# SunBangjie/FYP-BidirectionalPathTracer

Hardware: AMD Instinct MI355X
Metric: Mrays/s + RMSE vs the scalar oracle, BDPT pass, Sponza-class scene 1920x1080 depth 8 (higher is better)
Workload: dtype f32

## Files before the change

### fyp-bidirectionalpathtracer_amd/csrc/api.cpp

```cpp
#include <hip/hip_runtime.h>

#include <cmath>
#include <cstdio>
#include <cstdlib>
#include <cstring>
#include <future>
#include <functional>
#include <atomic>
#include <chrono>
#include <string>
#include <thread>
#include <vector>

#include "../../include/bdpt.h"
#include <new>

#include "bvh.h"
#include "kernels.h"
#include "refit.h"
#include "scene_bvh.h"

using namespace bdpt;

namespace {
// ... 440 lines not shown
    up(&u.shade, shade.data(), shade.size());
    up(&u.indices, d->indices, (size_t)d->numTriangles * 3);
    if (d->bitangents) up(&u.bitangents, d->bitangents, (size_t)d->numVertices * 3);
    return u;
  });
  struct SideJoin {
    std::future<SideUploads>& f;
    ~SideJoin() {
      if (!f.valid()) return;
      try {
        SideUploads u = f.get();
        for (void* q : u.pool) (void)hipFree(q);
      } catch (...) {
      }
    }
  } sideJoin{side};
  SceneBvh sb;
  try {
    std::string treeError;
    struct Build {
      BvhDeviceBuild* b;
      ~Build() { bvhDeviceBuildEnd(b); }
    } build{bvhDeviceBuildBegin(c->device, std::getenv("BDPT_HOST_COLLAPSE") == nullptr)};
    buildSceneBvh(d, 0, -1.0f, -1.0f, std::getenv("BDPT_NO_ALPHA_CLASSIFY") == nullptr, sb, buildBinaryTreeOnDevice, build.b, &treeError, packOnDevice, makeReferencesOnDevice,
                  std::getenv("BDPT_HOST_COLLAPSE") == nullptr, std::getenv("BDPT_HOST_PRIORITIES") == nullptr);
    if (sb.bvh.deviceRecs) c->sceneAllocs.push_back(sb.bvh.deviceRecs);
    if (!treeError.empty()) {
      fail(c, "scene: " + treeError);
      return treeError.find("2^31") != std::string::npos ? BDPT_E_LIMIT : (treeError.find("out of device memory") != std::string::npos ? BDPT_E_NOMEM : BDPT_E_HIP);
    }
  } catch (const std::bad_alloc&) {
    fail(c, "scene: out of host memory while building the acceleration structure");
    return BDPT_E_NOMEM;
  }
  lap("buildSceneBvh");
  Bvh& bvh = sb.bvh;
  const std::vector<uint32_t>& alphaTris = sb.alphaTris;
  if (bvh.maxStack > (uint32_t)kBvhMaxStack) {
    fail(c, "bvh needs a deeper traversal stack than the device provides");
    return BDPT_E_LIMIT;
  }
  if (!bvh.deviceRecs && !bvh.recs.empty()) {
    const BvhRec* dRecs = nullptr;
    if (int rc0 = devUpload(c, c->sceneAllocs, &dRecs, bvh.recs.data(), bvh.recs.size())) return rc0;
    bvh.deviceRecs = const_cast<BvhRec*>(dRecs);
    bvh.deviceNumRecs = bvh.recs.size();
  }
  if (!bvh.deviceRecs) {
    fail(c, "scene: the acceleration structure has no records");
    return BDPT_E_HIP;
  }
  c->bvhInfo.numNodes = bvh.numNodes;
  c->bvhInfo.numTriangles = d->numTriangles;
  c->bvhInfo.maxDepth = bvh.maxDepth;
  c->bvhInfo.nodeBytes = sizeof(BvhRec);
  c->bvhInfo.triBytes = sizeof(BvhTri);
  c->bvhInfo.sahCost = bvh.sahCost;
  c->bvhInfo.maxStack = bvh.maxStack;
  c->bvhInfo.numReferences = bvh.numRefs;
  c->bvhInfo.numDropped = bvh.numDropped;
  c->bvhInfo.numAlphaMode = sb.numAlphaMode;
  c->bvhInfo.numAlwaysPass = sb.numAlwaysPass;

  int rc;
  {
    SideUploads u = side.get();
    c->sceneAllocs.insert(c->sceneAllocs.end(), u.pool.begin(), u.pool.end());
    if (u.err != hipSuccess) {
      fail(c, std::string("scene upload: ") + (u.what.empty() ? std::string(hipGetErrorString(u.err)) : u.what));
      return u.err == hipErrorOutOfMemory ? BDPT_E_NOMEM : BDPT_E_HIP;
    }
    c->S.shade = reinterpret_cast<const float4*>(u.shade);
    c->S.indices = u.indices;
    if (d->bitangents) {
      c->S.bitangents = u.bitangents;
      c->S.hasBitangents = 1;
    }
  }
  lap("shading records + uploads (joined)");
  c->S.recs = reinterpret_cast<const uint4*>(bvh.deviceRecs);
  c->S.numRecs = (uint32_t)bvh.deviceNumRecs;
  if ((rc = devUpload(c, c->sceneAllocs, &c->S.materials, d->materials, d->numMaterials))) return rc;
  std::vector<TexDev> texs(d->numTextures);
  for (uint32_t i = 0; i < d->numTextures; i++) {
    const bdpt_texture& t = d->textures[i];
    if (!t.rgba8 || !t.width || !t.height) {
      fail(c, "scene: empty texture");
      return BDPT_E_INVALID;
    }
    const size_t bytes = (size_t)t.width * t.height * 4;
    uint8_t* px = nullptr;
    if ((rc = devAlloc(c, c->sceneAllocs, &px, bytes + 4))) return rc;
    HIPCHK(c, hipMemset(px + bytes, 0, 4));
    {
      std::string e;
      if (!bvhUploadStaged(px, t.rgba8, bytes, e)) {
        fail(c, e);
        return BDPT_E_HIP;
      }
    }
    texs[i] = TexDev{px, t.width, t.height, t.srgb, texPow2Flags(t.width, t.height)};
  }
  if ((rc = devUpload(c, c->sceneAllocs, &c->S.textures, texs.data(), texs.size()))) return rc;
  {
    std::vector<TexDev> matTex((size_t)d->numMaterials * 4, TexDev{nullptr, 0, 0, 0, 0});
    for (uint32_t mi = 0; mi < d->numMaterials; mi++) {
      const bdpt_material& mm = d->materials[mi];
      const int ids[4] = {mm.texBaseColor, mm.texSpecular, mm.texEmissive, mm.texNormal};
      for (int k = 0; k < 4; k++)
        if (ids[k] >= 0) matTex[(size_t)mi * 4 + k] = texs[(size_t)ids[k]];
    }
    if ((rc = devUpload(c, c->sceneAllocs, &c->S.matTex, matTex.data(), matTex.size()))) return rc;
  }
  {
    float4* dAlpha = nullptr;
    if ((rc = devAlloc(c, c->sceneAllocs, &dAlpha, std::max<size_t>(alphaTris.size(), 1) * 4))) return rc;
    if (alphaTris.empty()) {
      HIPCHK(c, hipMemset(dAlpha, 0, 4 * sizeof(float4)));
    } else {
      std::vector<uint8_t> alphaMat(d->numMaterials, 0);
      for (const uint32_t t : alphaTris) alphaMat[d->triMaterial[t]] = 1;
      std::vector<unsigned long long> quadByTex(std::max<size_t>(d->numTextures, 1), 0ull);
      for (uint32_t mi = 0; mi < d->numMaterials; mi++) {
        const bdpt_material& mm = d->materials[mi];
        if (!alphaMat[mi] || !alphaSamplesTexture(BDPT_FLAG_DIFFUSE_TYPE(mm.flags), mm.texBaseColor) || quadByTex[(size_t)mm.texBaseColor])
          continue;
        const std::vector<uint32_t> plane = alphaQuadPlane(d->textures[mm.texBaseColor]);
        const uint32_t* dPlane = nullptr;
        if ((rc = devUpload(c, c->sceneAllocs, &dPlane, plane.data(), plane.size()))) return rc;
        quadByTex[(size_t)mm.texBaseColor] = (unsigned long long)reinterpret_cast<uintptr_t>(dPlane);
      }
      const uint32_t* dList = nullptr;
      const unsigned long long* dQuad = nullptr;
      std::vector<void*> scratch;
      if ((rc = devUpload(c, c->sceneAllocs, &dList, alphaTris.data(), alphaTris.size())) ||
          (rc = devUpload(c, scratch, &dQuad, quadByTex.data(), quadByTex.size()))) {
        freePool(scratch);
        return rc;
      }
      c->alphaTris = dList;
      c->numAlphaTris = (uint32_t)alphaTris.size();
      launchAlphaRecs(c->S, dList, (uint32_t)alphaTris.size(), dQuad, dAlpha, nullptr);
      const hipError_t e = hipDeviceSynchronize();
      freePool(scratch);
      HIPCHK(c, e);
    }
    c->S.alphaRecs = dAlpha;
  }
  lap("indices, textures, alpha");
  SceneConst sc;
  std::memset(&sc, 0, sizeof(sc));
  std::memcpy(sc.lights, d->lights, sizeof(bdpt_light) * d->numLights);
  for (int i = 0; i < 256; i++) {
    double cc = (double)i / 255.0;
    double l = (cc <= 0.04045) ? cc / 12.92 : std::pow((cc + 0.055) / 1.055, 2.4);
    sc.srgbLut[i] = (float)l;
  }
  if ((rc = devUpload(c, c->sceneAllocs, &c->S.sc, &sc, 1))) return rc;
  c->S.numLights = d->numLights;
  c->hints = std::getenv("BDPT_NO_HINTS") == nullptr;
  if (c->hints) {
    uint32_t res = 512;
    if (const char* e = std::getenv("BDPT_LIGHT_MAP_RES")) res = (uint32_t)std::max(0, std::min(2048, std::atoi(e)));
    if (res) {
      uint32_t* maps = nullptr;
      if ((rc = devAlloc(c, c->sceneAllocs, &maps, (size_t)6 * res * res * d->numLights))) return rc;
      launchLightMaps(c->S, maps, res, nullptr);
      HIPCHK(c, hipDeviceSynchronize());
      c->S.lightMap = maps;
      c->S.lightMapRes = res;
      c->lightMaps = maps;
    }
  }
  if (c->hintPix) HIPCHK(c, hipMemset(c->hintPix, 0xFF, (size_t)c->W * c->H * sizeof(uint32_t)));
  c->hintCamValid = false;
  lap("light maps");
  c->numVertices = d->numVertices;
  c->numTriangles = d->numTriangles;
  c->haveScene = true;
  return BDPT_OK;
}
int bdpt_set_scene(bdpt_ctx* c, const bdpt_scene_desc* d) {
  try {
    return setSceneImpl(c, d);
  } catch (const std::bad_alloc&) {
    fail(c, "scene: out of host memory while building the acceleration structure");
    return BDPT_E_NOMEM;
  } catch (const std::exception& e) {
    fail(c, std::string("scene: ") + e.what());
    return BDPT_E_INVALID;
  }
}


int bdpt_get_bvh_info(const bdpt_ctx* c, bdpt_bvh_info* out) {
  if (!c || !out) return BDPT_E_INVALID;
  if (!c->haveScene) return BDPT_E_STATE;
  *out = c->bvhInfo;
  return BDPT_OK;
}

int bdpt_set_camera(bdpt_ctx* c, const bdpt_camera* cam) {
  if (!c || !cam) return BDPT_E_INVALID;
  c->cam = *cam;
  c->haveCamera = true;
  return BDPT_OK;
}

int bdpt_set_environment(bdpt_ctx* c, const bdpt_environment* env) {
  if (!c) return BDPT_E_INVALID;
  if (env && env->envMap && (!env->width || !env->height)) {
    fail(c, "environment: a map needs a width and a height");
    return BDPT_E_INVALID;
  }
  c->env = env ? *env : bdpt_environment{};
  if (!c->env.envMap) c->env.width = c->env.height = 0;
  return BDPT_OK;
}

namespace {
int ensureRefit(bdpt_ctx* c, hipStream_t st) {
  if (c->refitReady) return BDPT_OK;
  if (streamIsCapturing(st)) {
    fail(c, "update: the first update needs bdpt_prepare(BDPT_PREPARE_REFIT) before stream capture");
    return BDPT_E_STATE;
  }
  HIPCHK(c, hipDeviceSynchronize());
  BvhRefitPlan plan;
  {
    std::vector<BvhRec> recs(c->S.numRecs);
    HIPCHK(c, hipMemcpy(recs.data(), c->S.recs, recs.size() * sizeof(BvhRec), hipMemcpyDeviceToHost));
    std::string err;
    if (!bvhRefitMakePlan(recs.data(), recs.size(), plan, err)) {
      fail(c, err);
      return BDPT_E_HIP;
    }
  }
  const size_t nn = std::max<size_t>(plan.nodes.size(), 1);
  RefitDev R{};
  const BvhRefitNode* dNodes = nullptr;
// ... 1440 lines not shown
```

### fyp-bidirectionalpathtracer_amd/csrc/device_scene.hpp

```cpp
#pragma once
#include "device_math.hpp"
#include "kernels.h"

namespace bdpt {
#define BD __device__ __forceinline__

struct f4 {
  float x, y, z, w;
};
BD f4 lerp4(f4 a, f4 b, float s) {
  return f4{a.x + (b.x - a.x) * s, a.y + (b.y - a.y) * s, a.z + (b.z - a.z) * s, a.w + (b.w - a.w) * s};
}
typedef __attribute__((address_space(1))) const uint32_t gU32;
typedef __attribute__((address_space(1), aligned(4))) const unsigned long long gU64a4;
BD void texelRow(const uint8_t* px, uint32_t w, int iy, int ix0, int ix1, uint32_t& a, uint32_t& b) {
  gU32* row = (gU32*)px + (size_t)iy * w;
  const unsigned long long q = *(gU64a4*)(row + ix0);
  a = (uint32_t)q;
  b = (uint32_t)(q >> 32);
  if (ix1 != ix0 + 1) b = row[ix1];
}
BD f4 texel(const SceneDev& S, const TexDev& t, uint32_t p) {
  f4 r;
  if (t.srgb) {
    r.x = S.sc->srgbLut[p & 0xffu];
    r.y = S.sc->srgbLut[(p >> 8) & 0xffu];
    r.z = S.sc->srgbLut[(p >> 16) & 0xffu];
  } else {
    r.x = (float)(p & 0xffu) / 255.0f;
    r.y = (float)((p >> 8) & 0xffu) / 255.0f;
    r.z = (float)((p >> 16) & 0xffu) / 255.0f;
  }
  r.w = (float)(p >> 24) / 255.0f;
  return r;
}
BD f4 sampleBilinearT(const SceneDev& S, const TexDev& t, float u, float v) {
  float x = u * (float)t.w - 0.5f;
  float y = v * (float)t.h - 0.5f;
  float x0 = floorf(x), y0 = floorf(y);
  float fx = x - x0, fy = y - y0;
  int ix0 = wrapT((int)x0, (int)t.w, (t.pow2 & kTexPow2W) != 0u), iy0 = wrapT((int)y0, (int)t.h, (t.pow2 & kTexPow2H) != 0u);
  int ix1 = wrapNext(ix0, (int)t.w), iy1 = wrapNext(iy0, (int)t.h);
  uint32_t p00, p10, p01, p11;
  texelRow(t.px, t.w, iy0, ix0, ix1, p00, p10);
  texelRow(t.px, t.w, iy1, ix0, ix1, p01, p11);
  f4 t00 = texel(S, t, p00), t10 = texel(S, t, p10);
  f4 t01 = texel(S, t, p01), t11 = texel(S, t, p11);
  return lerp4(lerp4(t00, t10, fx), lerp4(t01, t11, fx), fy);
}
BD f4 sampleBilinear(const SceneDev& S, int texId, float u, float v) { return sampleBilinearT(S, S.textures[texId], u, v); }
BD f4 sampleTexture(const SceneDev& S, int texId, float u, float v, f4 factor, uint32_t mode) {
  if (mode == BDPT_CHANNEL_UNUSED) return f4{0, 0, 0, 0};
  if (mode == BDPT_CHANNEL_CONST || texId < 0) return factor;
  return sampleBilinear(S, texId, u, v);
}
BD f4 sampleTextureT(const SceneDev& S, const TexDev& t, int texId, float u, float v, f4 factor, uint32_t mode) {
  if (mode == BDPT_CHANNEL_UNUSED) return f4{0, 0, 0, 0};
  if (mode == BDPT_CHANNEL_CONST || texId < 0) return factor;
  return sampleBilinearT(S, t, u, v);
}

struct MatDev {
  f4 baseColor, specular;
  f3 emissive;
  float alphaThreshold, IoR;
  uint32_t flags;
  int texBase, texSpec, texEmis, texNorm;
};
BD MatDev loadMaterial(const SceneDev& S, uint32_t id) {
  const float4* m = reinterpret_cast<const float4*>(S.materials + id);
  float4 a = m[0], b = m[1], c = m[2], d = m[3];
  MatDev r;
  r.baseColor = f4{a.x, a.y, a.z, a.w};
  r.specular = f4{b.x, b.y, b.z, b.w};
  r.emissive = mk(c.x, c.y, c.z);
  r.alphaThreshold = c.w;
  r.IoR = d.x;
  r.flags = __float_as_uint(d.y);
  uint32_t t0 = __float_as_uint(d.z), t1 = __float_as_uint(d.w);
  r.texBase = (int)(int16_t)(t0 & 0xffffu);
  r.texSpec = (int)(int16_t)(t0 >> 16);
  r.texEmis = (int)(int16_t)(t1 & 0xffffu);
  r.texNorm = (int)(int16_t)(t1 >> 16);
  return r;
}

BD uint32_t alphaQuad(const float4& a2, const float4& a3, float u, float v, float& fx, float& fy) {
  const int tw = (int)__float_as_uint(a2.y), th = (int)__float_as_uint(a2.z);
  const uint32_t pow2 = __float_as_uint(a2.w);
  gU32* px = (gU32*)(((unsigned long long)__float_as_uint(a3.y) << 32) | (unsigned long long)__float_as_uint(a3.x));
  const float x = u * (float)tw - 0.5f, y = v * (float)th - 0.5f;
  const float x0 = floorf(x), y0 = floorf(y);
  fx = x - x0;
  fy = y - y0;
  const int ix0 = wrapT((int)x0, tw, (pow2 & kTexPow2W) != 0u), iy0 = wrapT((int)y0, th, (pow2 & kTexPow2H) != 0u);
  return px[(size_t)iy0 * tw + (size_t)ix0];
}
BD bool alphaTestFails(const SceneDev& S, uint32_t rec, float bu, float bv) {
  const float4* r = S.alphaRecs + (size_t)rec * 4;
  const float4 a0 = r[0], a1 = r[1], a2 = r[2], a3 = r[3];
  const uint32_t mode = __float_as_uint(a2.x);
  float alpha = 0.0f;
  if (mode == 1u) {
    alpha = a1.w;
  } else if (mode == 2u) {
    float u = 0, v = 0;
    const float b0 = 1.0f - bu - bv;
    u += a0.x * b0;
    v += a0.y * b0;
    u += a0.z * bu;
    v += a0.w * bu;
    u += a1.x * bv;
    v += a1.y * bv;
    float fx, fy;
    const uint32_t q = alphaQuad(a2, a3, u, v, fx, fy);
    const float t00 = (float)(q & 0xffu) / 255.0f, t10 = (float)((q >> 8) & 0xffu) / 255.0f;
    const float t01 = (float)((q >> 16) & 0xffu) / 255.0f, t11 = (float)(q >> 24) / 255.0f;
    const float top = t00 + (t10 - t00) * fx, bot = t01 + (t11 - t01) * fx;
    alpha = top + (bot - top) * fy;
  }
  return alpha < a1.z;
}

struct AlphaIn {
  float4 a0, a1, a2, a3;
};
BD void alphaTexels(const AlphaIn& r, float bu, float bv, bool run, float& fx, float& fy, float& t00, float& t10, float& t01, float& t11) {
  fx = fy = t00 = t10 = t01 = t11 = 0.0f;
  if (!run || __float_as_uint(r.a2.x) != 2u) return;
  float u = 0, v = 0;
  const float b0 = 1.0f - bu - bv;
  u += r.a0.x * b0;
  v += r.a0.y * b0;
  u += r.a0.z * bu;
  v += r.a0.w * bu;
  u += r.a1.x * bv;
  v += r.a1.y * bv;
  const uint32_t q = alphaQuad(r.a2, r.a3, u, v, fx, fy);
  t00 = (float)(q & 0xffu);
  t10 = (float)((q >> 8) & 0xffu);
  t01 = (float)((q >> 16) & 0xffu);
  t11 = (float)(q >> 24);
}
BD bool alphaVerdict(const AlphaIn& r, float fx, float fy, float t00, float t10, float t01, float t11) {
  const uint32_t mode = __float_as_uint(r.a2.x);
  float alpha = 0.0f;
  if (mode == 1u) {
    alpha = r.a1.w;
  } else if (mode == 2u) {
    const float w00 = t00 / 255.0f, w10 = t10 / 255.0f, w01 = t01 / 255.0f, w11 = t11 / 255.0f;
    const float top = w00 + (w10 - w00) * fx, bot = w01 + (w11 - w01) * fx;
    alpha = top + (bot - top) * fy;
  }
  return alpha < r.a1.z;
}
BD void alphaTestFails2(const SceneDev& S, bool need0, uint32_t rec0, float u0, float v0, bool need1, uint32_t rec1, float u1, float v1,
                        bool& fail0, bool& fail1) {
  AlphaIn r0, r1;
  r0.a0 = r0.a1 = r0.a2 = r0.a3 = r1.a0 = r1.a1 = r1.a2 = r1.a3 = make_float4(0.0f, 0.0f, 0.0f, 0.0f);
  if (need0) {
    const float4* p = S.alphaRecs + (size_t)rec0 * 4;
    r0.a0 = p[0];
    r0.a1 = p[1];
    r0.a2 = p[2];
    r0.a3 = p[3];
  }
  if (need1) {
    const float4* p = S.alphaRecs + (size_t)rec1 * 4;
    r1.a0 = p[0];
    r1.a1 = p[1];
    r1.a2 = p[2];
    r1.a3 = p[3];
  }
  float fx0, fy0, a00, a10, a01, a11, fx1, fy1, b00, b10, b01, b11;
  alphaTexels(r0, u0, v0, need0, fx0, fy0, a00, a10, a01, a11);
  alphaTexels(r1, u1, v1, need1, fx1, fy1, b00, b10, b01, b11);
  fail0 = need0 && alphaVerdict(r0, fx0, fy0, a00, a10, a01, a11);
  fail1 = need1 && alphaVerdict(r1, fx1, fy1, b00, b10, b01, b11);
}

struct Shading {
  f3 posW, V, N, diffuse, specular, emissive;
  float opacity, linearRoughness, roughness, IoR;
};
template <bool NMAP>
BD Shading shadeHit(const SceneDev& S, uint32_t prim, float bu, float bv, f3 camPosW) {
  const float4* r = S.shade + (size_t)prim * kShadeRecF4;
  const float4 r0 = r[0], r1 = r[1], r2 = r[2], r3 = r[3], r4 = r[4], r5 = r[5], r6 = r[6];
  const float b0 = 1.0f - bu - bv;
  float u = 0, v = 0;
  f3 normalW = mk(0), posW = mk(0);
  u += r1.z * b0;
  v += r1.w * b0;
  normalW = normalW + mk(r0.w, r1.x, r1.y) * b0;
  posW = posW + mk(r0.x, r0.y, r0.z) * b0;
  u += r3.z * bu;
  v += r3.w * bu;
  normalW = normalW + mk(r2.w, r3.x, r3.y) * bu;
  posW = posW + mk(r2.x, r2.y, r2.z) * bu;
  u += r5.z * bv;
  v += r5.w * bv;
  normalW = normalW + mk(r4.w, r5.x, r5.y) * bv;
  posW = posW + mk(r4.x, r4.y, r4.z) * bv;
  normalW = normalize(normalW);

  const uint32_t matId = __float_as_uint(r6.x);
  const MatDev m = loadMaterial(S, matId);
  const TexDev tBase = S.matTex[(size_t)matId * 4], tSpec = S.matTex[(size_t)matId * 4 + 1], tEmis = S.matTex[(size_t)matId * 4 + 2];
  Shading sd;
  f4 base = sampleTextureT(S, tBase, m.texBase, u, v, m.baseColor, BDPT_FLAG_DIFFUSE_TYPE(m.flags));
  sd.opacity = m.baseColor.w;
  sd.posW = posW;
  sd.V = normalize(camPosW - posW);
  sd.N = normalize(normalW);
  f4 spec = sampleTextureT(S, tSpec, m.texSpec, u, v, m.specular, BDPT_FLAG_SPECULAR_TYPE(m.flags));
  f3 baseRgb = mk(base.x, base.y, base.z);
  if (BDPT_FLAG_SHADING_MODEL(m.flags) == BDPT_SHADING_MODEL_METAL_ROUGH) {
    sd.diffuse = lerp3(baseRgb, mk(0), spec.z);
    sd.specular = lerp3(mk(0.04f), baseRgb, spec.z);
    sd.linearRoughness = spec.y;
  } else {
    sd.diffuse = baseRgb;
    sd.specular = mk(spec.x, spec.y, spec.z);
    sd.linearRoughness = 1.0f - spec.w;
  }
  sd.linearRoughness = maxf(0.08f, sd.linearRoughness);
  sd.roughness = sd.linearRoughness * sd.linearRoughness;
  f4 em = sampleTextureT(S, tEmis, m.texEmis, u, v, f4{m.emissive.x, m.emissive.y, m.emissive.z, 1.0f}, BDPT_FLAG_EMISSIVE_TYPE(m.flags));
  sd.emissive = mk(em.x, em.y, em.z);
  sd.IoR = m.IoR;
  const bool doubleSided = BDPT_FLAG_DOUBLE_SIDED(m.flags) != 0;
  if (NMAP) {
    const uint32_t mapType = BDPT_FLAG_NORMAL_MAP_TYPE(m.flags);
    if (mapType != BDPT_NORMAL_MAP_UNUSED && m.texNorm >= 0 && S.hasBitangents) {
      f3 bitW = mk(0);
      const float bw[3] = {b0, bu, bv};
#pragma unroll
      for (int i = 0; i < 3; i++) {
        uint32_t vi = S.indices[(size_t)prim * 3 + i];
        bitW = bitW + ld3(S.bitangents + (size_t)vi * 3) * bw[i];
      }
      bitW = normalize(bitW);
      f3 B = normalize(bitW - sd.N * dot(bitW, sd.N));
      f3 T = normalize(cross(B, sd.N));
      f4 mp = sampleBilinear(S, m.texNorm, u, v);
      f3 mapN;
      if (mapType == BDPT_NORMAL_MAP_RGB) {
        mapN = normalize(mk(mp.x, mp.y, mp.z) * 2.0f - mk(1.0f));
      } else {
        float nx = mp.x * 2.0f - 1.0f, ny = mp.y * 2.0f - 1.0f;
        float nz = saturate(mp.x * mp.x + mp.y * mp.y);
        nz = sqrtf(1.0f - nz);
        mapN = normalize(mk(nx, ny, nz));
      }
      sd.N = T * mapN.x + B * mapN.y + sd.N * mapN.z;
    }
  }
  float NdotV = dot(sd.N, sd.V);
  if (NdotV <= 0.0f && doubleSided) sd.N = -sd.N;
  return sd;
}

BD void primaryRay(const bdpt_camera& cam, const bdpt_gbuffer_params& gp, uint32_t x, uint32_t y, uint32_t W, uint32_t H, f3& o, f3& d) {
  const f3 U = ld3(cam.cameraU), V = ld3(cam.cameraV), Wv = ld3(cam.cameraW), camPos = ld3(cam.posW);
  float pcx = ((float)x + gp.pixelJitter[0]) / (float)W;
  float pcy = ((float)y + gp.pixelJitter[1]) / (float)H;
  float ndx = 2.0f * pcx + -1.0f;
  float ndy = -2.0f * pcy + 1.0f;
  f3 rayDir = U * ndx + V * ndy + Wv;
  rayDir = rayDir / length(Wv);
  f3 focalPoint = camPos + rayDir * gp.focalLen;
  uint32_t randSeed = initRand(x + y * W, gp.frameCount);
  float r0 = nextRand(randSeed);
  float r1 = nextRand(randSeed);
  float sn, cs;
  det_sincos2pi(r0, sn, cs);
  float lr = gp.lensRadius * r1;
  float lu = cs * lr, lv = sn * lr;
  f3 randomOrig = camPos + normalize(U) * lu + normalize(V) * lv;
  o = gp.useThinLens ? randomOrig : camPos;
  d = normalize(gp.useThinLens ? (focalPoint - randomOrig) : rayDir);
}

#undef BD
}
```

### fyp-bidirectionalpathtracer_amd/csrc/kernels.h

```cpp
#pragma once
#include <hip/hip_runtime.h>
#include <stdint.h>

#include "../../include/bdpt.h"
#include "texture_planes.h"

namespace bdpt {

constexpr int kWave = 64;
#ifndef KSTACK
#define KSTACK 32
#endif
constexpr int kStackEntries = KSTACK;
#ifndef BDPT_STACK_LDS
#define BDPT_STACK_LDS 24
#endif
constexpr int kStackLds = BDPT_STACK_LDS < KSTACK ? BDPT_STACK_LDS : KSTACK;
constexpr int kMaxPersistentPerCU = 32;
constexpr int kStackOvfRows = KSTACK - kStackLds;
constexpr int kShadeRecF4 = 7;
constexpr uint32_t kNoRay = 0xFFFFFFFFu;
constexpr uint32_t kNumSubQueues = 32;
#ifndef BDPT_FETCH_CHUNK
#define BDPT_FETCH_CHUNK 256
#endif
constexpr uint32_t kFetchChunk = BDPT_FETCH_CHUNK;
constexpr uint32_t kCursorStride = 32;
constexpr uint32_t kCursorBlock = kNumSubQueues * kCursorStride;
#ifndef BDPT_RAY_SUBQUEUES
#define BDPT_RAY_SUBQUEUES 32
#endif
constexpr uint32_t kNumRaySubQueues = BDPT_RAY_SUBQUEUES;
constexpr uint32_t kRayCursorBlock = kNumRaySubQueues * kCursorStride;
constexpr uint32_t kCounterShards = 64;

enum : int { F_COL = 0, F_POS = 3, F_N = 6, F_V = 9, F_DIF = 12, F_SPEC = 15, F_ROUGH = 18, F_ISSPEC = 19, F_PDF = 20, NF = 21 };
constexpr int NF4 = 6;
enum : int { PATH_EYE = 0, PATH_LIGHT = 1 };
enum : int { RAY_TERMS = 0, RAY_PAIRS = 1 };

struct TexDev {
  const uint8_t* px;
  uint32_t w, h, srgb, pow2;
};

struct SceneConst {
  bdpt_light lights[BDPT_MAX_LIGHTS];
  float srgbLut[256];
};

struct SceneDev {
  const uint4* recs;
  const float4* shade;
  const float* bitangents;
  const uint32_t* indices;
  const bdpt_material* materials;
  const TexDev* textures;
  const TexDev* matTex;
  const SceneConst* sc;
  uint32_t numLights;
  uint32_t hasBitangents;
  uint32_t numRecs;
  const float4* alphaRecs;
  int* stackOvf;
  uint32_t stackOvfStride;
  const uint32_t* lightMap;
  uint32_t lightMapRes;
};

struct DevCounters {
  unsigned long long v[kCounterShards][32];
};
enum : int {
  C_RAYS_PRIMARY = 0, C_RAYS_EYE, C_RAYS_LIGHT, C_RAYS_NEE, C_RAYS_SPLAT, C_RAYS_CONNECT,
  C_NODE_CLOSEST, C_TRI_CLOSEST, C_NODE_SHADOW, C_TRI_SHADOW, C_PIX_VALID, C_SPLATS, C_RAYS_LAZY,
  C_STACK_MAX,
  C_ALPHA_CLOSEST, C_ALPHA_SHADOW,
  C_HINT_NEE, C_HINT_SPLAT
};

inline __host__ __device__ uint32_t numConnectPairs(uint32_t D) {
  uint32_t n = 0;
  for (uint32_t t = 2; t <= D; t++) n += (t < D - 1) ? t : (D - 1);
  return n;
}

struct PathBuf {
  float* v;
  float* rayDir;
  const uint32_t* pix;
  uint32_t* seedE;
  uint32_t* seedL;
  uint8_t* eyeLast;
  uint8_t* lightLast;
  uint8_t* lightReal;
  uint32_t* queue[3];
  uint32_t pathSubCap;
  uint32_t* qcount;
  uint32_t* qhead;
  float* rayQ;
  float* rayContrib;
  uint8_t* rayVis;
  uint32_t* rayCount;
  uint32_t* rayHead;
  uint32_t raySubCap[2];
  uint32_t rayBase[2];
  uint32_t* slotRay;
  uint32_t* splatPix;
  float* misE;
  float* misL;
  uint8_t* lazyCursor;
  uint32_t* lazyRay;
  uint32_t* lazyCount;
  uint32_t rayCap;
  uint32_t Np, D1;
};

struct SplatLayout {
  uint32_t stripeRows, owners, chunkRows;
};
inline __host__ __device__ size_t splatIndex(const SplatLayout& L, uint32_t W, uint32_t x, uint32_t y) {
  const uint32_t s = y / L.stripeRows;
  const uint32_t owner = s % L.owners, row = (s / L.owners) * L.stripeRows + (y - s * L.stripeRows);
  return ((size_t)owner * L.chunkRows + row) * W + x;
}

struct FrameDev {
  bdpt_camera cam;
  bdpt_params p;
  uint32_t W, H;
  SplatLayout sl;
  float* out;
  unsigned long long* splat;
  bdpt_gbuffer gb;
  DevCounters* counters;
  const float* envMap;
  uint32_t envW, envH;
  float envColor[3];
  const uint32_t* hintPix;
};

struct GroupDev {
  float* planes;
  unsigned long long* splat;
  uint8_t* lightIdx;
  uint32_t numLights;
  uint64_t framePix;
};

struct MaskDev {
  const uint8_t* mask;
  uint32_t* eye;
  uint32_t* eyeCount;
  const uint32_t* walkEye;
  const uint32_t* walkEyeCount;
};

constexpr uint32_t kNoAlphaRec = 0xFFFFFFFFu;
struct BvhRefitNode;
struct AreaDev {
  const float* cdf;
  const float4* emit;
  const float* total;
  uint32_t n;
};

enum class FrameKind { Plain, Groups, Masked };
struct FrameVariant {
  FrameKind kind = FrameKind::Plain;
  GroupDev groups{};
  MaskDev mask{};
  AreaDev area{};
};

struct GBufferDev {
  bdpt_camera cam;
  bdpt_gbuffer_params gp;
  uint32_t W, H, Np;
  const uint32_t* pix;
  bdpt_gbuffer gb;
  DevCounters* counters;
  uint32_t* hintPix;
};

struct BmfrDev {
  uint32_t W, H, frame;
  uint32_t full, doPre;
  float m[16];
  const float4* curPos;
  const uint16_t* curNorm;
  const uint16_t* albedo;
  float4* noisy;
  const float4 *prevPosR, *prevNormR, *prevNoisyR, *prevFilteredR;
  float4 *prevPosW, *prevNormW, *prevNoisyW, *prevFilteredW;
  uint8_t* accept;
  uint32_t* prevPixel;
};
void launchBmfr(const BmfrDev& A, uint32_t flags, hipStream_t st);

void launchGBuffer(const SceneDev& S, const GBufferDev& G, hipStream_t st);
void launchAlphaRecs(const SceneDev& S, const uint32_t* alphaTris, uint32_t n, const unsigned long long* quadByTex, float4* out, hipStream_t st);
void launchHintFill(const SceneDev& S, const GBufferDev& G, hipStream_t st);
void launchLightMaps(const SceneDev& S, uint32_t* maps, uint32_t res, hipStream_t st);
void launchInitPaths(const SceneDev& S, const FrameDev& F, const PathBuf& P, const FrameVariant& V, hipStream_t st);
struct LaunchGrids {
  uint32_t walk[16] = {};
  uint32_t shadow[2] = {0, 0};
  uint32_t rays[3] = {0, 0, 0};
};
void launchWalk(const SceneDev& S, const FrameDev& F, const PathBuf& P, const FrameVariant& V, LaunchGrids& G, int numCUs,
                hipStream_t st);
void launchMisPrefix(const FrameDev& F, const PathBuf& P, hipStream_t st);
void launchGenNee(const SceneDev& S, const FrameDev& F, const PathBuf& P, const AreaDev& A, hipStream_t st);
void launchGenSplat(const SceneDev& S, const FrameDev& F, const PathBuf& P, hipStream_t st);
void launchGenConnect(const SceneDev& S, const FrameDev& F, const PathBuf& P, hipStream_t st);
void launchTraceShadow(const SceneDev& S, const FrameDev& F, const PathBuf& P, int rayClass, LaunchGrids& G, int numCUs, hipStream_t st);
void launchTraceRays(const SceneDev& S, const float4* rays, uint32_t cap, const uint32_t* count, unsigned long long* cursor, int mode,
                     float4* hits, uint8_t* vis, LaunchGrids& G, int numCUs, hipStream_t st);
void launchCameraRays(const bdpt_camera& cam, const bdpt_gbuffer_params& gp, uint32_t W, uint32_t H, float4* rays, hipStream_t st);
void launchShadeHits(const SceneDev& S, uint32_t numTris, const float4* rays, const float4* hits, uint32_t cap, const uint32_t* count,
                     bool normalMap, float4* out, hipStream_t st);
void launchBsdfQuery(const float4* surf, uint32_t cap, const uint32_t* count, bool eval, bool ggx, bool fromLobe, const uint32_t* seeds,
                     const float4* dirs, float4* out, hipStream_t st);
void launchGather(const FrameDev& F, const PathBuf& P, const FrameVariant& V, uint32_t* lazyList, uint32_t* lazyCount, hipStream_t st);
void launchLazyGen(const FrameDev& F, const PathBuf& P, const uint32_t* list, const uint32_t* listCount, int batch, hipStream_t st);
void launchLazyCheck(const FrameDev& F, const PathBuf& P, const FrameVariant& V, const uint32_t* list, const uint32_t* listCount,
                     int batch, uint32_t* nextList, uint32_t* nextCount, hipStream_t st);
constexpr int kLazyBatchDiv = 8;
constexpr int kMaxLazyRounds = 8;
void launchResolve(const unsigned long long* splat, bool tileLocal, uint32_t splatRow0, const SplatLayout& L, float* out, uint32_t W,
                   const uint32_t* pix, uint32_t Np, hipStream_t st);
void launchFrameResolve(const FrameDev& F, const PathBuf& P, const FrameVariant& V, hipStream_t st);
struct AdaptiveDev {
  float4* mean;
  float* m2;
  uint32_t* count;
  uint8_t* mask;
  uint32_t* active;
  float4* frame;
  uint32_t W, H;
  float threshold, epsilon;
  uint32_t minSamples, maxSamples, blockSize;
};
void launchAdaptiveUpdate(const AdaptiveDev& A, unsigned long long* scratch, hipStream_t st);
void launchAdaptiveReset(const AdaptiveDev& A, hipStream_t st);
void launchAccumulate(float* last, float* cur, uint32_t accumCount, uint32_t maxAccum, uint64_t numTexels, hipStream_t st);
void launchAccumulateTile(float* last, float* cur, uint32_t accumCount, uint32_t maxAccum, const uint32_t* pix, uint32_t Np,
                          hipStream_t st);
void launchTilePack(const void* frame, void* packed, uint32_t bytesPerPixel, const uint32_t* pix, uint32_t Np, hipStream_t st);
void launchTileUnpack(const void* packed, void* frame, uint32_t bytesPerPixel, uint32_t W, uint32_t H, uint32_t stripeRows, uint32_t owners,
                      uint32_t owner, uint32_t packedRows, hipStream_t st);
void launchTestRng(const uint32_t* v0, const uint32_t* v1, uint32_t n, uint32_t draws, uint32_t* states, float* floats,
                   hipStream_t st);
void launchTestTrace(const SceneDev& S, const float* rays, uint32_t n, int mode, int32_t* prim, float* tuv, hipStream_t st);
void launchTestTraceShadow(const SceneDev& S, const float* planes, uint32_t cap, const uint32_t* count, uint32_t* head, uint8_t* vis,
                           DevCounters* counters, float tmin, int numCUs, hipStream_t st);
void launchTestBsdf(const float* in, uint32_t n, uint32_t matIndex, float* out, hipStream_t st);

void launchAreaMarkReferenced(const BvhRefitNode* nodes, uint32_t numNodes, const uint4* recs, uint8_t* referenced, hipStream_t st);
void launchAreaCount(const SceneDev& S, uint32_t numTris, const uint8_t* referenced, uint32_t* blockCount, uint32_t* blockBase,
                     uint32_t* counts, hipStream_t st);
void launchAreaCompact(const SceneDev& S, uint32_t numTris, const uint8_t* referenced, const uint32_t* blockBase,
                       const uint32_t* alphaTris, uint32_t numAlphaTris, float4* emit, hipStream_t st);
void launchAreaRefresh(const SceneDev& S, const AreaDev& A, float* blockSum, uint32_t* blockLast, hipStream_t st);
void launchTestAreaSample(const SceneDev& S, const AreaDev& A, int mode, const uint32_t* states, const float* points, uint32_t n,
                          float* out, hipStream_t st);

}
```

### fyp-bidirectionalpathtracer_amd/csrc/kernels.hip

```cpp
#include "kernels.h"

#include <algorithm>
#include <type_traits>

#include "device_area.hpp"
#include "device_math.hpp"
#include "device_scene.hpp"
#include "device_trace.hpp"
#include "launch.hpp"

namespace bdpt {

#define BD __device__ __forceinline__

BD void wavePush(bool active, uint32_t value, uint32_t* items, uint32_t* count, uint32_t subCap, uint32_t q = 0xffffffffu) {
  unsigned long long mask = __ballot(active);
  if (mask == 0ull) return;
  const int lane = (int)(threadIdx.x & 63u);
  const int leader = __ffsll((long long)mask) - 1;
  if (q == 0xffffffffu) q = blockIdx.x % kNumSubQueues;
  uint32_t base = 0;
  if (lane == leader) base = atomicAdd(&count[q * kCursorStride], (uint32_t)__popcll(mask));
  base = (uint32_t)__shfl((int)base, leader);
  const uint32_t prefix = (uint32_t)__popcll(mask & ((1ull << lane) - 1ull));
// ... 1421 lines not shown
  f3 N = ld3(p), V = ld3(p + 3), Lq = ld3(p + 6), dif = ld3(p + 9), spec = ld3(p + 12);
  float rough = p[15];
  bool isSpec = p[16] != 0.0f;
  uint32_t seed = __float_as_uint(p[17]);
  f3 L;
  float pdf;
  bool sSpec;
  f3 w = sampleBRDF<GGX>(seed, N, N, V, dif, spec, rough, fromLobe, L, pdf, sSpec);
  f3 fr = evalBRDF<GGX>(V, Lq, N, N, dif, spec, rough, isSpec);
  float* o = out + (size_t)i * 16;
  o[0] = w.x;
  o[1] = w.y;
  o[2] = w.z;
  o[3] = L.x;
  o[4] = L.y;
  o[5] = L.z;
  o[6] = pdf;
  o[7] = sSpec ? 1.0f : 0.0f;
  o[8] = fr.x;
  o[9] = fr.y;
  o[10] = fr.z;
  o[11] = o[12] = o[13] = o[14] = o[15] = 0.0f;
}


static inline uint32_t blocksFor(uint64_t n) { return (uint32_t)((n + kWave - 1) / kWave); }
static inline uint32_t queueGrid(const PathBuf& P) { return (P.pathSubCap / kWave) * kNumSubQueues; }


template <class Fn>
static void withFlags(Fn&& fn) {
  fn();
}
template <class Fn, class... Flags>
static void withFlags(Fn&& fn, bool f, Flags... rest) {
  if (f)
    withFlags([&](auto... t) { fn(std::true_type{}, t...); }, rest...);
  else
    withFlags([&](auto... t) { fn(std::false_type{}, t...); }, rest...);
}
template <class Fn>
static void withKind(FrameKind kind, Fn&& fn) {
  if (kind == FrameKind::Groups)
    fn(std::integral_constant<FrameKind, FrameKind::Groups>{});
  else if (kind == FrameKind::Masked)
    fn(std::integral_constant<FrameKind, FrameKind::Masked>{});
  else
    fn(std::integral_constant<FrameKind, FrameKind::Plain>{});
}
template <FrameKind K>
static FrameArg<K> frameArg(const FrameVariant& V) {
  if constexpr (K == FrameKind::Groups)
    return V.groups;
  else if constexpr (K == FrameKind::Masked)
    return V.mask;
  else
    return NoArg{};
}

void launchGBuffer(const SceneDev& S, const GBufferDev& G, hipStream_t st) {
  const uint32_t Np = G.Np;
  if (!Np) return;
  withFlags([&](auto CNT) { launchWave(gbuffer_kernel<CNT>, blocksFor(Np), st, S, G); }, G.counters != nullptr);
}

__global__ void alpha_recs_kernel(SceneDev S, const uint32_t* __restrict__ alphaTris, uint32_t n, const unsigned long long* __restrict__ quadByTex,
                                  float4* __restrict__ out) {
  const uint32_t i = blockIdx.x * blockDim.x + threadIdx.x;
  if (i >= n) return;
  const uint32_t t = alphaTris[i];
  const float4* sr = S.shade + (size_t)t * kShadeRecF4;
  const float4 a1 = sr[1], b1 = sr[3], c1 = sr[5], m6 = sr[6];
  const uint32_t mid = __float_as_uint(m6.x);
  const bdpt_material& m = S.materials[mid];
  const uint32_t type = BDPT_FLAG_DIFFUSE_TYPE(m.flags);
  uint32_t mode = 0, tw = 0, th = 0, pow2 = 0;
  unsigned long long px = 0;
  if (type == BDPT_CHANNEL_UNUSED) {
    mode = 0;
  } else if (!alphaSamplesTexture(type, m.texBaseColor)) {
    mode = 1;
  } else {
    mode = 2;
    const TexDev td = S.matTex[(size_t)mid * 4];
    tw = td.w;
    th = td.h;
    pow2 = td.pow2;
    px = quadByTex[m.texBaseColor];
  }
  float4* r = out + (size_t)i * 4;
  r[0] = make_float4(a1.z, a1.w, b1.z, b1.w);
  r[1] = make_float4(c1.z, c1.w, m.alphaThreshold, m.baseColor[3]);
  r[2] = make_float4(__uint_as_float(mode), __uint_as_float(tw), __uint_as_float(th), __uint_as_float(pow2));
  r[3] = make_float4(__uint_as_float((uint32_t)(px & 0xffffffffull)), __uint_as_float((uint32_t)(px >> 32)), 0.0f, 0.0f);
}
void launchAlphaRecs(const SceneDev& S, const uint32_t* alphaTris, uint32_t n, const unsigned long long* quadByTex, float4* out, hipStream_t st) {
  if (!n) return;
  hipLaunchKernelGGL(alpha_recs_kernel, dim3((n + 255) / 256), dim3(256), 0, st, S, alphaTris, n, quadByTex, out);
}

void launchHintFill(const SceneDev& S, const GBufferDev& G, hipStream_t st) {
  if (!G.Np || !G.hintPix) return;
  launchWave(gbuffer_kernel<false, true>, (uint32_t)(blocksFor(G.Np)), st, S, G);
}

void launchLightMaps(const SceneDev& S, uint32_t* maps, uint32_t res, hipStream_t st) {
  const uint64_t n = (uint64_t)6 * res * res * S.numLights;
  if (!n) return;
  launchWave(light_map_kernel, (uint32_t)((n + kWave - 1) / kWave), st, S, maps, res);
}

void launchInitPaths(const SceneDev& S, const FrameDev& F, const PathBuf& P, const FrameVariant& V, hipStream_t st) {
  if (!P.Np) return;
  if (V.area.n && V.kind != FrameKind::Groups) {
    const bool masked = V.kind == FrameKind::Masked;
    withFlags(
        [&](auto GGX, auto MASKED) {
          constexpr FrameKind K = MASKED ? FrameKind::Masked : FrameKind::Plain;
          launchWave(init_paths_area_kernel<GGX, K>, blocksFor(P.Np), st, S, F, P, frameArg<K>(V), V.area);
        },
        F.p.matIndex == 0, masked);
    return;
  }
  withKind(V.kind, [&](auto K) {
    withFlags([&](auto GGX) { launchWave(init_paths_kernel<GGX, K>, blocksFor(P.Np), st, S, F, P, frameArg<K>(V)); }, F.p.matIndex == 0);
  });
}

void launchWalk(const SceneDev& S, const FrameDev& F, const PathBuf& P, const FrameVariant& V, LaunchGrids& G, int numCUs,
                hipStream_t st) {
  if (!P.Np || F.p.maxDepth < 1) return;
  const bool cnt = (F.p.flags & BDPT_PARAM_COUNTERS) != 0, ggx = F.p.matIndex == 0;
  const bool ext = (F.p.flags & (BDPT_PARAM_ENV_ON_MISS | BDPT_PARAM_EMISSIVE_HITS)) != 0, masked = V.kind == FrameKind::Masked;
  uint32_t& g = G.walk[(masked ? 8 : 0) + (ext ? 4 : 0) + (ggx ? 2 : 0) + (cnt ? 1 : 0)];
  const uint32_t need = blocksFor((uint64_t)2 * P.Np);
  withFlags(
      [&](auto GGX, auto CNT, auto EXT, auto MASKED) {
        const auto kernel = walk_kernel<GGX, CNT, EXT, MASKED>;
        if (!g) g = persistentGrid(kernel, numCUs);
        launchWave(kernel, std::min(g, need), st, S, F, P, P.qhead, frameArg<MASKED ? FrameKind::Masked : FrameKind::Plain>(V));
      },
      ggx, cnt, ext, masked);
}

void launchMisPrefix(const FrameDev& F, const PathBuf& P, hipStream_t st) {
  if (!P.Np) return;
  launchWave(mis_prefix_kernel, (uint32_t)(queueGrid(P)), st, F, P);
}
void launchGenNee(const SceneDev& S, const FrameDev& F, const PathBuf& P, const AreaDev& A, hipStream_t st) {
  if (!P.Np) return;
  if (A.n) {
    withFlags([&](auto GGX, auto WIDE) { launchWave(gen_nee_area_kernel<GGX, WIDE ? 16 : 8>, queueGrid(P) * (WIDE ? 16 : 8), st, S, F, P, A); },
              F.p.matIndex == 0, P.D1 > 9);
    return;
  }
  withFlags([&](auto GGX, auto WIDE) { launchWave(gen_nee_kernel<GGX, WIDE ? 16 : 8>, queueGrid(P) * (WIDE ? 16 : 8), st, S, F, P); },
            F.p.matIndex == 0, P.D1 > 9);
}
void launchGenSplat(const SceneDev& S, const FrameDev& F, const PathBuf& P, hipStream_t st) {
  if (!P.Np || (F.p.flags & BDPT_PARAM_NO_SPLAT)) return;
  withFlags([&](auto GGX, auto WIDE) { launchWave(gen_splat_kernel<GGX, WIDE ? 16 : 8>, queueGrid(P) * (WIDE ? 16 : 8), st, S, F, P); },
            F.p.matIndex == 0, P.D1 > 9);
}
void launchGenConnect(const SceneDev& S, const FrameDev& F, const PathBuf& P, hipStream_t st) {
  if (!P.Np || (F.p.flags & BDPT_PARAM_NO_CONNECT) || F.p.maxDepth < 2) return;
  withFlags([&](auto GGX, auto WIDE) { launchWave(gen_connect_kernel<GGX, WIDE ? 16 : 8>, queueGrid(P) * (WIDE ? 16 : 8), st, S, F, P); },
            F.p.matIndex == 0, P.D1 > 9);
}

void launchTraceShadow(const SceneDev& S, const FrameDev& F, const PathBuf& P, int cls, LaunchGrids& G, int numCUs, hipStream_t st) {
  if (!P.Np) return;
  const bool cnt = (F.p.flags & BDPT_PARAM_COUNTERS) != 0;
  RayQueue Q{P.rayQ + P.rayBase[cls], P.rayCap, P.raySubCap[cls], kNumRaySubQueues, P.rayCount + (size_t)cls * kRayCursorBlock,
             P.rayHead + (size_t)cls * kRayCursorBlock};
  uint8_t* vis = P.rayVis + P.rayBase[cls];
  uint32_t& g = G.shadow[cnt ? 1 : 0];
  withFlags(
      [&](auto CNT) {
        if (!g) g = persistentGrid(trace_shadow_kernel<CNT>, numCUs);
        launchWave(trace_shadow_kernel<CNT>, g, st, S, Q, vis, F.counters, F.p.minT);
      },
// ... 119 lines not shown
```

### fyp-bidirectionalpathtracer_amd/csrc/texture_planes.h

```cpp
#pragma once
#include <stddef.h>
#include <stdint.h>

#include "../../include/bdpt.h"

#if defined(__HIPCC__)
#define BDPT_HD __host__ __device__ inline
#else
#define BDPT_HD inline
#endif

namespace bdpt {

enum : uint32_t { kTexPow2W = 1u, kTexPow2H = 2u };
BDPT_HD uint32_t texPow2Flags(uint32_t w, uint32_t h) {
  return ((w & (w - 1u)) == 0u ? kTexPow2W : 0u) | ((h & (h - 1u)) == 0u ? kTexPow2H : 0u);
}

BDPT_HD int wrapi(int i, int n) {
  int m = i % n;
  return (m < 0) ? m + n : m;
}
BDPT_HD int wrapT(int i, int n, bool pow2) { return pow2 ? (i & (n - 1)) : wrapi(i, n); }
BDPT_HD int wrapNext(int i, int n) { return (i + 1 == n) ? 0 : i + 1; }

BDPT_HD bool alphaSamplesTexture(uint32_t diffuseType, int texBaseColor) {
  return diffuseType != BDPT_CHANNEL_UNUSED && diffuseType != BDPT_CHANNEL_CONST && texBaseColor >= 0;
}

inline void alphaQuadRows(const uint8_t* rgba8, uint32_t w, uint32_t h, uint32_t y0, uint32_t y1, uint32_t* out) {
  for (uint32_t y = y0; y < y1; y++) {
    const uint32_t yn = (uint32_t)wrapNext((int)y, (int)h);
    for (uint32_t x = 0; x < w; x++) {
      const uint32_t xn = (uint32_t)wrapNext((int)x, (int)w);
      const uint32_t a00 = rgba8[((size_t)y * w + x) * 4 + 3], a10 = rgba8[((size_t)y * w + xn) * 4 + 3];
      const uint32_t a01 = rgba8[((size_t)yn * w + x) * 4 + 3], a11 = rgba8[((size_t)yn * w + xn) * 4 + 3];
      out[(size_t)y * w + x] = a00 | (a10 << 8) | (a01 << 16) | (a11 << 24);
    }
  }
}

}
```

Baseline: 4841.

## Pre-decode textures to float4 planes and inline texture descriptors in material records

```diff
diff --git a/fyp-bidirectionalpathtracer_amd/csrc/api.cpp b/fyp-bidirectionalpathtracer_amd/csrc/api.cpp
--- a/fyp-bidirectionalpathtracer_amd/csrc/api.cpp
+++ b/fyp-bidirectionalpathtracer_amd/csrc/api.cpp
@@ -546,35 +546,67 @@
   c->S.numRecs = (uint32_t)bvh.deviceNumRecs;
   if ((rc = devUpload(c, c->sceneAllocs, &c->S.materials, d->materials, d->numMaterials))) return rc;
   std::vector<TexDev> texs(d->numTextures);
-  for (uint32_t i = 0; i < d->numTextures; i++) {
-    const bdpt_texture& t = d->textures[i];
-    if (!t.rgba8 || !t.width || !t.height) {
-      fail(c, "scene: empty texture");
-      return BDPT_E_INVALID;
-    }
-    const size_t bytes = (size_t)t.width * t.height * 4;
-    uint8_t* px = nullptr;
-    if ((rc = devAlloc(c, c->sceneAllocs, &px, bytes + 4))) return rc;
-    HIPCHK(c, hipMemset(px + bytes, 0, 4));
-    {
-      std::string e;
-      if (!bvhUploadStaged(px, t.rgba8, bytes, e)) {
-        fail(c, e);
-        return BDPT_E_HIP;
+  {
+    std::vector<void*> scratch;
+    struct Free {
+      std::vector<void*>& p;
+      ~Free() { freePool(p); }
+    } freeScratch{scratch};
+    float tables[kTexelTableSize];
+    texelTables(tables);
+    const float* dTables = nullptr;
+    if (d->numTextures && (rc = devUpload(c, scratch, &dTables, tables, (size_t)kTexelTableSize))) return rc;
+    for (uint32_t i = 0; i < d->numTextures; i++) {
+      const bdpt_texture& t = d->textures[i];
+      if (!t.rgba8 || !t.width || !t.height) {
+        fail(c, "scene: empty texture");
+        return BDPT_E_INVALID;
       }
-    }
-    texs[i] = TexDev{px, t.width, t.height, t.srgb, texPow2Flags(t.width, t.height)};
+      const size_t n = (size_t)t.width * t.height;
+      const uint32_t* bytes = nullptr;
+      float4* plane = nullptr;
+      if ((rc = devUpload(c, scratch, &bytes, reinterpret_cast<const uint32_t*>(t.rgba8), n)) || (rc = devAlloc(c, c->sceneAllocs, &plane, n)))
+        return rc;
+      launchDecodeTexels(bytes, n, t.srgb != 0, dTables, plane, nullptr);
+      texs[i] = TexDev{plane, t.width, t.height, texPow2Flags(t.width, t.height), 0u};
+    }
+    HIPCHK(c, hipDeviceSynchronize());
   }
   if ((rc = devUpload(c, c->sceneAllocs, &c->S.textures, texs.data(), texs.size()))) return rc;
   {
-    std::vector<TexDev> matTex((size_t)d->numMaterials * 4, TexDev{nullptr, 0, 0, 0, 0});
+    std::vector<float> recs((size_t)d->numMaterials * 32, 0.0f);
+    auto word = [](uint32_t v) {
+      float f;
+      std::memcpy(&f, &v, 4);
+      return f;
+    };
     for (uint32_t mi = 0; mi < d->numMaterials; mi++) {
       const bdpt_material& mm = d->materials[mi];
-      const int ids[4] = {mm.texBaseColor, mm.texSpecular, mm.texEmissive, mm.texNormal};
-      for (int k = 0; k < 4; k++)
-        if (ids[k] >= 0) matTex[(size_t)mi * 4 + k] = texs[(size_t)ids[k]];
-    }
-    if ((rc = devUpload(c, c->sceneAllocs, &c->S.matTex, matTex.data(), matTex.size()))) return rc;
+      float* r = recs.data() + (size_t)mi * 32;
+      std::memcpy(r, mm.baseColor, 16);
+      std::memcpy(r + 4, mm.specular, 16);
+      std::memcpy(r + 8, mm.emissive, 12);
+      r[11] = mm.alphaThreshold;
+      r[12] = mm.IoR;
+      r[13] = word(mm.flags);
+      r[14] = word((uint32_t)(int32_t)mm.texNormal);
+      const int ids[3] = {mm.texBaseColor, mm.texSpecular, mm.texEmissive};
+      uint32_t pow2 = 0;
+      for (int k = 0; k < 3; k++) {
+        if (ids[k] < 0) continue;
+        const TexDev& t = texs[(size_t)ids[k]];
+        const unsigned long long px = (unsigned long long)reinterpret_cast<uintptr_t>(t.px);
+        r[16 + 4 * k] = word((uint32_t)(px & 0xffffffffull));
+        r[17 + 4 * k] = word((uint32_t)(px >> 32));
+        r[18 + 4 * k] = word(t.w);
+        r[19 + 4 * k] = word(t.h);
+        pow2 |= t.pow2 << (2 * k);
+      }
+      r[15] = word(pow2);
+    }
+    const float* dRecs = nullptr;
+    if ((rc = devUpload(c, c->sceneAllocs, &dRecs, recs.data(), recs.size()))) return rc;
+    c->S.matRecs = reinterpret_cast<const float4*>(dRecs);
   }
   {
     float4* dAlpha = nullptr;
@@ -615,11 +647,6 @@
   SceneConst sc;
   std::memset(&sc, 0, sizeof(sc));
   std::memcpy(sc.lights, d->lights, sizeof(bdpt_light) * d->numLights);
-  for (int i = 0; i < 256; i++) {
-    double cc = (double)i / 255.0;
-    double l = (cc <= 0.04045) ? cc / 12.92 : std::pow((cc + 0.055) / 1.055, 2.4);
-    sc.srgbLut[i] = (float)l;
-  }
   if ((rc = devUpload(c, c->sceneAllocs, &c->S.sc, &sc, 1))) return rc;
   c->S.numLights = d->numLights;
   c->hints = std::getenv("BDPT_NO_HINTS") == nullptr;
diff --git a/fyp-bidirectionalpathtracer_amd/csrc/device_scene.hpp b/fyp-bidirectionalpathtracer_amd/csrc/device_scene.hpp
--- a/fyp-bidirectionalpathtracer_amd/csrc/device_scene.hpp
+++ b/fyp-bidirectionalpathtracer_amd/csrc/device_scene.hpp
@@ -12,64 +12,55 @@
   return f4{a.x + (b.x - a.x) * s, a.y + (b.y - a.y) * s, a.z + (b.z - a.z) * s, a.w + (b.w - a.w) * s};
 }
 typedef __attribute__((address_space(1))) const uint32_t gU32;
-typedef __attribute__((address_space(1), aligned(4))) const unsigned long long gU64a4;
-BD void texelRow(const uint8_t* px, uint32_t w, int iy, int ix0, int ix1, uint32_t& a, uint32_t& b) {
-  gU32* row = (gU32*)px + (size_t)iy * w;
-  const unsigned long long q = *(gU64a4*)(row + ix0);
-  a = (uint32_t)q;
-  b = (uint32_t)(q >> 32);
-  if (ix1 != ix0 + 1) b = row[ix1];
-}
-BD f4 texel(const SceneDev& S, const TexDev& t, uint32_t p) {
-  f4 r;
-  if (t.srgb) {
-    r.x = S.sc->srgbLut[p & 0xffu];
-    r.y = S.sc->srgbLut[(p >> 8) & 0xffu];
-    r.z = S.sc->srgbLut[(p >> 16) & 0xffu];
-  } else {
-    r.x = (float)(p & 0xffu) / 255.0f;
-    r.y = (float)((p >> 8) & 0xffu) / 255.0f;
-    r.z = (float)((p >> 16) & 0xffu) / 255.0f;
-  }
-  r.w = (float)(p >> 24) / 255.0f;
-  return r;
-}
-BD f4 sampleBilinearT(const SceneDev& S, const TexDev& t, float u, float v) {
+typedef float texel4 __attribute__((ext_vector_type(4)));
+typedef __attribute__((address_space(1))) const texel4 gTexel4;
+BD f4 sampleBilinearT(const TexDev& t, float u, float v) {
   float x = u * (float)t.w - 0.5f;
   float y = v * (float)t.h - 0.5f;
   float x0 = floorf(x), y0 = floorf(y);
   float fx = x - x0, fy = y - y0;
   int ix0 = wrapT((int)x0, (int)t.w, (t.pow2 & kTexPow2W) != 0u), iy0 = wrapT((int)y0, (int)t.h, (t.pow2 & kTexPow2H) != 0u);
   int ix1 = wrapNext(ix0, (int)t.w), iy1 = wrapNext(iy0, (int)t.h);
-  uint32_t p00, p10, p01, p11;
-  texelRow(t.px, t.w, iy0, ix0, ix1, p00, p10);
-  texelRow(t.px, t.w, iy1, ix0, ix1, p01, p11);
-  f4 t00 = texel(S, t, p00), t10 = texel(S, t, p10);
-  f4 t01 = texel(S, t, p01), t11 = texel(S, t, p11);
+  gTexel4* row0 = (gTexel4*)t.px + (size_t)iy0 * t.w;
+  gTexel4* row1 = (gTexel4*)t.px + (size_t)iy1 * t.w;
+  const texel4 q00 = row0[ix0], q10 = row0[ix1], q01 = row1[ix0], q11 = row1[ix1];
+  f4 t00 = f4{q00.x, q00.y, q00.z, q00.w}, t10 = f4{q10.x, q10.y, q10.z, q10.w};
+  f4 t01 = f4{q01.x, q01.y, q01.z, q01.w}, t11 = f4{q11.x, q11.y, q11.z, q11.w};
   return lerp4(lerp4(t00, t10, fx), lerp4(t01, t11, fx), fy);
 }
-BD f4 sampleBilinear(const SceneDev& S, int texId, float u, float v) { return sampleBilinearT(S, S.textures[texId], u, v); }
+BD f4 sampleBilinear(const SceneDev& S, int texId, float u, float v) { return sampleBilinearT(S.textures[texId], u, v); }
 BD f4 sampleTexture(const SceneDev& S, int texId, float u, float v, f4 factor, uint32_t mode) {
   if (mode == BDPT_CHANNEL_UNUSED) return f4{0, 0, 0, 0};
   if (mode == BDPT_CHANNEL_CONST || texId < 0) return factor;
   return sampleBilinear(S, texId, u, v);
 }
-BD f4 sampleTextureT(const SceneDev& S, const TexDev& t, int texId, float u, float v, f4 factor, uint32_t mode) {
+BD f4 sampleTextureT(const TexDev& t, float u, float v, f4 factor, uint32_t mode) {
   if (mode == BDPT_CHANNEL_UNUSED) return f4{0, 0, 0, 0};
-  if (mode == BDPT_CHANNEL_CONST || texId < 0) return factor;
-  return sampleBilinearT(S, t, u, v);
-}
-
+  if (mode == BDPT_CHANNEL_CONST || !t.px) return factor;
+  return sampleBilinearT(t, u, v);
+}
+
+constexpr int kMatRecF4 = 8;
 struct MatDev {
   f4 baseColor, specular;
   f3 emissive;
   float alphaThreshold, IoR;
   uint32_t flags;
-  int texBase, texSpec, texEmis, texNorm;
-};
+  int texNorm;
+  TexDev tBase, tSpec, tEmis;
+};
+BD TexDev matChannel(const float4& c, uint32_t pow2) {
+  TexDev t;
+  t.px = (const float4*)(((unsigned long long)__float_as_uint(c.y) << 32) | (unsigned long long)__float_as_uint(c.x));
+  t.w = __float_as_uint(c.z);
+  t.h = __float_as_uint(c.w);
+  t.pow2 = pow2 & 3u;
+  t.pad = 0u;
+  return t;
+}
 BD MatDev loadMaterial(const SceneDev& S, uint32_t id) {
-  const float4* m = reinterpret_cast<const float4*>(S.materials + id);
-  float4 a = m[0], b = m[1], c = m[2], d = m[3];
+  const float4* m = S.matRecs + (size_t)id * kMatRecF4;
+  const float4 a = m[0], b = m[1], c = m[2], d = m[3], tb = m[4], ts = m[5], te = m[6];
   MatDev r;
   r.baseColor = f4{a.x, a.y, a.z, a.w};
   r.specular = f4{b.x, b.y, b.z, b.w};
@@ -77,11 +68,11 @@
   r.alphaThreshold = c.w;
   r.IoR = d.x;
   r.flags = __float_as_uint(d.y);
-  uint32_t t0 = __float_as_uint(d.z), t1 = __float_as_uint(d.w);
-  r.texBase = (int)(int16_t)(t0 & 0xffffu);
-  r.texSpec = (int)(int16_t)(t0 >> 16);
-  r.texEmis = (int)(int16_t)(t1 & 0xffffu);
-  r.texNorm = (int)(int16_t)(t1 >> 16);
+  r.texNorm = (int)__float_as_uint(d.z);
+  const uint32_t pow2 = __float_as_uint(d.w);
+  r.tBase = matChannel(tb, pow2);
+  r.tSpec = matChannel(ts, pow2 >> 2);
+  r.tEmis = matChannel(te, pow2 >> 4);
   return r;
 }
 
@@ -206,14 +197,13 @@
 
   const uint32_t matId = __float_as_uint(r6.x);
   const MatDev m = loadMaterial(S, matId);
-  const TexDev tBase = S.matTex[(size_t)matId * 4], tSpec = S.matTex[(size_t)matId * 4 + 1], tEmis = S.matTex[(size_t)matId * 4 + 2];
   Shading sd;
-  f4 base = sampleTextureT(S, tBase, m.texBase, u, v, m.baseColor, BDPT_FLAG_DIFFUSE_TYPE(m.flags));
+  f4 base = sampleTextureT(m.tBase, u, v, m.baseColor, BDPT_FLAG_DIFFUSE_TYPE(m.flags));
   sd.opacity = m.baseColor.w;
   sd.posW = posW;
   sd.V = normalize(camPosW - posW);
   sd.N = normalize(normalW);
-  f4 spec = sampleTextureT(S, tSpec, m.texSpec, u, v, m.specular, BDPT_FLAG_SPECULAR_TYPE(m.flags));
+  f4 spec = sampleTextureT(m.tSpec, u, v, m.specular, BDPT_FLAG_SPECULAR_TYPE(m.flags));
   f3 baseRgb = mk(base.x, base.y, base.z);
   if (BDPT_FLAG_SHADING_MODEL(m.flags) == BDPT_SHADING_MODEL_METAL_ROUGH) {
     sd.diffuse = lerp3(baseRgb, mk(0), spec.z);
@@ -226,7 +216,7 @@
   }
   sd.linearRoughness = maxf(0.08f, sd.linearRoughness);
   sd.roughness = sd.linearRoughness * sd.linearRoughness;
-  f4 em = sampleTextureT(S, tEmis, m.texEmis, u, v, f4{m.emissive.x, m.emissive.y, m.emissive.z, 1.0f}, BDPT_FLAG_EMISSIVE_TYPE(m.flags));
+  f4 em = sampleTextureT(m.tEmis, u, v, f4{m.emissive.x, m.emissive.y, m.emissive.z, 1.0f}, BDPT_FLAG_EMISSIVE_TYPE(m.flags));
   sd.emissive = mk(em.x, em.y, em.z);
   sd.IoR = m.IoR;
   const bool doubleSided = BDPT_FLAG_DOUBLE_SIDED(m.flags) != 0;
diff --git a/fyp-bidirectionalpathtracer_amd/csrc/kernels.h b/fyp-bidirectionalpathtracer_amd/csrc/kernels.h
--- a/fyp-bidirectionalpathtracer_amd/csrc/kernels.h
+++ b/fyp-bidirectionalpathtracer_amd/csrc/kernels.h
@@ -40,13 +40,12 @@
 enum : int { RAY_TERMS = 0, RAY_PAIRS = 1 };
 
 struct TexDev {
-  const uint8_t* px;
-  uint32_t w, h, srgb, pow2;
+  const float4* px;
+  uint32_t w, h, pow2, pad;
 };
 
 struct SceneConst {
   bdpt_light lights[BDPT_MAX_LIGHTS];
-  float srgbLut[256];
 };
 
 struct SceneDev {
@@ -56,7 +55,7 @@
   const uint32_t* indices;
   const bdpt_material* materials;
   const TexDev* textures;
-  const TexDev* matTex;
+  const float4* matRecs;
   const SceneConst* sc;
   uint32_t numLights;
   uint32_t hasBitangents;
@@ -200,6 +199,7 @@
 
 void launchGBuffer(const SceneDev& S, const GBufferDev& G, hipStream_t st);
 void launchAlphaRecs(const SceneDev& S, const uint32_t* alphaTris, uint32_t n, const unsigned long long* quadByTex, float4* out, hipStream_t st);
+void launchDecodeTexels(const uint32_t* rgba8, size_t n, bool srgb, const float* tables, float4* plane, hipStream_t st);
 void launchHintFill(const SceneDev& S, const GBufferDev& G, hipStream_t st);
 void launchLightMaps(const SceneDev& S, uint32_t* maps, uint32_t res, hipStream_t st);
 void launchInitPaths(const SceneDev& S, const FrameDev& F, const PathBuf& P, const FrameVariant& V, hipStream_t st);
diff --git a/fyp-bidirectionalpathtracer_amd/csrc/kernels.hip b/fyp-bidirectionalpathtracer_amd/csrc/kernels.hip
--- a/fyp-bidirectionalpathtracer_amd/csrc/kernels.hip
+++ b/fyp-bidirectionalpathtracer_amd/csrc/kernels.hip
@@ -1527,7 +1527,7 @@
     mode = 1;
   } else {
     mode = 2;
-    const TexDev td = S.matTex[(size_t)mid * 4];
+    const TexDev td = S.textures[m.texBaseColor];
     tw = td.w;
     th = td.h;
     pow2 = td.pow2;
@@ -1542,6 +1542,22 @@
 void launchAlphaRecs(const SceneDev& S, const uint32_t* alphaTris, uint32_t n, const unsigned long long* quadByTex, float4* out, hipStream_t st) {
   if (!n) return;
   hipLaunchKernelGGL(alpha_recs_kernel, dim3((n + 255) / 256), dim3(256), 0, st, S, alphaTris, n, quadByTex, out);
+}
+
+__global__ void decode_texels_kernel(const uint32_t* __restrict__ rgba8, size_t n, bool srgb, const float* __restrict__ tables,
+                                     float4* __restrict__ plane) {
+  __shared__ float lds[kTexelTableSize];
+  for (uint32_t k = threadIdx.x; k < kTexelTableSize; k += blockDim.x) lds[k] = tables[k];
+  __syncthreads();
+  const size_t i = (size_t)blockIdx.x * blockDim.x + threadIdx.x;
+  if (i >= n) return;
+  float t[4];
+  decodeTexel(rgba8[i], srgb, lds, t);
+  plane[i] = make_float4(t[0], t[1], t[2], t[3]);
+}
+void launchDecodeTexels(const uint32_t* rgba8, size_t n, bool srgb, const float* tables, float4* plane, hipStream_t st) {
+  if (!n) return;
+  hipLaunchKernelGGL(decode_texels_kernel, dim3((uint32_t)((n + 255) / 256)), dim3(256), 0, st, rgba8, n, srgb, tables, plane);
 }
 
 void launchHintFill(const SceneDev& S, const GBufferDev& G, hipStream_t st) {
diff --git a/fyp-bidirectionalpathtracer_amd/csrc/texture_planes.h b/fyp-bidirectionalpathtracer_amd/csrc/texture_planes.h
--- a/fyp-bidirectionalpathtracer_amd/csrc/texture_planes.h
+++ b/fyp-bidirectionalpathtracer_amd/csrc/texture_planes.h
@@ -1,4 +1,5 @@
 #pragma once
+#include <math.h>
 #include <stddef.h>
 #include <stdint.h>
 
@@ -40,4 +41,25 @@
   }
 }
 
+BDPT_HD float texelChannel(uint32_t b, bool srgb) {
+  if (!srgb) return (float)b / 255.0f;
+  const double cc = (double)b / 255.0;
+  const double l = (cc <= 0.04045) ? cc / 12.92 : pow((cc + 0.055) / 1.055, 2.4);
+  return (float)l;
 }
+enum : uint32_t { kTexelTableLinear = 0u, kTexelTableSrgb = 256u, kTexelTableSize = 512u };
+inline void texelTables(float* tables) {
+  for (uint32_t b = 0; b < 256u; b++) {
+    tables[kTexelTableLinear + b] = texelChannel(b, false);
+    tables[kTexelTableSrgb + b] = texelChannel(b, true);
+  }
+}
+BDPT_HD void decodeTexel(uint32_t p, bool srgb, const float* tables, float* out) {
+  const float* rgb = tables + (srgb ? kTexelTableSrgb : kTexelTableLinear);
+  out[0] = rgb[p & 0xffu];
+  out[1] = rgb[(p >> 8) & 0xffu];
+  out[2] = rgb[(p >> 16) & 0xffu];
+  out[3] = tables[kTexelTableLinear + (p >> 24)];
+}
+
+}
```

Measured after the change: 4822. Within noise of the previous version (-0.4%).
